# taintpro98/rnd-semantic-segmentation

Measured on AMD Instinct MI355X. Metric: train images/sec at 769x769 bf16 (DeepLabV2-ResNet101 + ASPP), higher is better.
Workload: dtype bf16; 1 GPU; train_src.py DeepLabV2-R101 bf16, 769x769 synthetic Cityscapes crops, batch 8 per GPU, 1xMI355X; global_batch=8, parallelism=dp1, weights=formula (synthetic), hip_graph_replay=False

## Files before the change

### __graft_entry__.py

```python
import os
import subprocess
import sys

ROOT = os.path.dirname(os.path.abspath(__file__))
PKG = os.path.join(ROOT, "rnd_semantic_segmentation_amd")
CSRC = os.path.join(PKG, "csrc")
LIB = os.path.join(PKG, "libmi355seg.so")
SOURCES = ["igemm_nt.hip", "igemm_pp.hip", "igemm_tn.hip", "igemm_f32.hip", "pack_aspp.hip", "upsample_ce.hip", "upsample_infer.hip", "elementwise.hip", "stem.hip", "fada.hip", "colsum.hip", "batchnorm.hip", "structure_loss.hip", "comm.hip", "gconv.hip", "gnet.hip", "gald.hip", "gf32.hip", "chain.hip", "augment.hip", "augment_pra.hip", "polyp_score.hip"]


def _headers():
    return [os.path.join(CSRC, f) for f in os.listdir(CSRC) if f.endswith(".h")] + [os.path.join(ROOT, "include", "mi355seg.h")]


def _compile_one(hipcc, src, obj):
    subprocess.run([hipcc, "--offload-arch=gfx950", "-O3", "-std=c++17", "-fPIC", "-Wno-unused-result", "-c", src, "-o", obj], check=True, cwd=CSRC)


def build(force=False):
    from concurrent.futures import ThreadPoolExecutor
    hipcc = os.environ.get("HIPCC", "/opt/rocm/bin/hipcc")
    objdir = os.path.join(ROOT, "build", "obj")
    os.makedirs(objdir, exist_ok=True)
    hdr_t = max(os.path.getmtime(h) for h in _headers())
    jobs, objs = [], []
    for s in SOURCES:
        src, obj = os.path.join(CSRC, s), os.path.join(objdir, s.replace(".hip", ".o"))
        objs.append(obj)
        if force or not os.path.exists(obj) or os.path.getmtime(obj) < max(os.path.getmtime(src), hdr_t):
            jobs.append((src, obj))
    if jobs:
        with ThreadPoolExecutor(max_workers=min(len(jobs), max(1, (os.cpu_count() or 2) - 1))) as ex:
            for f in [ex.submit(_compile_one, hipcc, a, b) for a, b in jobs]:
                f.result()
    if jobs or not os.path.exists(LIB) or os.path.getmtime(LIB) < max(os.path.getmtime(o) for o in objs):
        subprocess.run([hipcc, "--offload-arch=gfx950", "-shared", "-fPIC", "-o", LIB] + objs + ["-ldl"], check=True, cwd=CSRC)
    if ROOT not in sys.path:
        sys.path.insert(0, ROOT)
    import rnd_semantic_segmentation_amd
    from rnd_semantic_segmentation_amd import _lib
    assert _lib.lib().mi_version() >= 100
# ... 47 lines not shown
```

### include/mi355seg.h

```cpp
#ifndef MI355SEG_H
#define MI355SEG_H

#include <stddef.h>
#include <stdint.h>

#ifdef __cplusplus
extern "C" {
#endif

#define MI355SEG_VERSION 100

#define MI_OK 0
#define MI_EINVAL (-22)
#define MI_ENOMEM (-12)
#define MI_EHIP (-5)

#define MI_EPI_SCALE_BIAS 1
#define MI_EPI_RESIDUAL 2
#define MI_EPI_RELU 4
#define MI_EPI_MASK 8
#define MI_EPI_OUT_F32 16
#define MI_EPI_ZSPLIT 32
#define MI_EPI_WRITE_MASK 64
#define MI_EPI_LEAKY 256
// ... 109 lines not shown
size_t mi_upsample_tversky_bce_workspace(int B, int h, int w, int H, int W);
int mi_upsample_tversky_bce(const float* low, const float* mask, float* loss_out , float* dlow, float* sums ,
                            int B, int h, int w, int H, int W, float alpha, float eps, float w_tversky, float w_bce, float grad_scale,
                            int align_corners, void* workspace, size_t workspace_bytes, void* stream);

int mi_upsample_softmax(const float* low, float* probs, uint8_t* pred, int B, int h, int w, int K, int H, int W, void* stream);

typedef struct { const float* low; int h, w; int mirror; } MiProbSource;
int mi_upsample_softmax_multi(const MiProbSource* src, int n, float* probs, int K, int H, int W, float div_a, float div_b, void* stream);

int mi_upsample_predict_score(const MiProbSource* src, int n, int K, int H, int W, float div_a, float div_b, const int64_t* labels,
                              int ignore_index, float threshold, uint8_t* pred, uint8_t* pseudo, int64_t* counts, void* stream);

int mi_upsample_predict_score_cw(const MiProbSource* src, int n, int K, int H, int W, float div_a, float div_b, const int64_t* labels,
                                 int ignore_index, const float* class_threshold, uint8_t* pred, uint8_t* pseudo, int64_t* counts, int bins,
                                 int64_t* hist, void* stream);

#define MI_POLYP_SUMS 24
#define MI_POLYP_COUNTS 4
size_t mi_polyp_score_workspace(int B, int h, int w, int H, int W);
int mi_polyp_score(const float* low, const int64_t* labels, int B, int h, int w, int H, int W, int64_t* hist, double* sums, int64_t* counts,
                   float* prob, uint8_t* pred, void* workspace, size_t workspace_bytes, void* stream);

int mi_image_resize_ac(const float* x, float* out, int B, int C, int H, int W, int Ho, int Wo, int with_mirror, void* stream);

int mi_sgd_step(float* p, const float* g, float* buf, size_t n, float lr, float momentum, float weight_decay, void* stream);
int mi_sgd_step_dev(float* p, const float* g, float* buf, size_t n, const float* hyper , void* stream);

int mi_stem_pool_fwd(const void* y, const float* scale, const float* shift, void* pool, uint8_t* idx,
                     int B, int Hc, int Wc, int C, int Hp, int Wp, void* stream);
int mi_stem_pool_bwd(const void* dpool, const uint8_t* idx, const float* scale, void* dy,
                     int B, int Hc, int Wc, int C, int Hp, int Wp, void* stream);
int mi_stem_im2col(const void* x_bf16_nhwc, void* col_bf16, int B, int H, int W, int Ho, int Wo, int ncols, void* stream);

int mi_bias_grad_bf16(const void* dy_bf16, float* db, int M, int N, int accumulate,
                      void* workspace , size_t workspace_bytes, void* stream);
size_t mi_upsample_softce_workspace(int B, int h, int w, int K, int H, int W);
int mi_upsample_softce(const float* seg_low, float inv_temperature, float clip, const float* d_low, int ldD, int domain,
                       float* loss_out, float* dd_low, int B, int h, int w, int K, int H, int W, float grad_scale,
                       void* workspace, size_t workspace_bytes, void* stream);
size_t mi_upsample_softce_2grid_workspace(int B, int hd, int wd, int K, int H, int W);
int mi_upsample_softce_2grid(const float* seg_low, int hs, int ws, int seg_align_corners, float inv_temperature, float clip,
                             const float* d_low, int hd, int wd, int ldD, int d_align_corners, int domain, float grad_scale,
                             float* loss_out, float* dd_low, int B, int K, int H, int W, void* workspace, size_t workspace_bytes, void* stream);
int mi_adam_step(float* p, const float* g, float* exp_avg, float* exp_avg_sq, size_t n, float lr, float beta1, float beta2,
                 float eps, int step, void* stream);
int mi_adam_step_clamped(float* p, float* g, float* exp_avg, float* exp_avg_sq, size_t n, float lr, float beta1, float beta2,
                         float eps, int step, float grad_clamp, void* stream);

int mi_adam_step_dev(float* p, float* g, float* exp_avg, float* exp_avg_sq, size_t n, const float* hyper , void* stream);

int mi_pack_weight_f32(const float* w_oihw, float* wp, int O, int I, int ksize, void* stream);
int mi_conv_f32(const float* a, const float* wp, float* out, int B, int Ha, int Wa, int Ca, int Ho, int Wo, int N,
                int ksize, int stride, int pad, int dil, const float* scale, const float* bias, const float* res,
                int flags, void* stream);
int mi_stem_f32(const float* x_nchw, const float* w, const float* scale, const float* shift, float* y_nhwc,
                int B, int H, int W, void* stream);
int mi_maxpool_f32(const float* y_nhwc, float* pool_nhwc, int B, int Hc, int Wc, int C, void* stream);

int mi_comm_unique_id(void* id128 );
int mi_comm_init_rank(void** comm , int nranks, const void* id128 , int rank);
int mi_comm_destroy(void* comm);
int mi_allreduce_bucket(void* ptr, size_t count, int dtype, int average, void* comm, void* stream);

int mi_relu_mask(const void* x_bf16, const void* msk, void* y_bf16, size_t n, int bits, void* stream);
int mi_frozen_bn_fold(const float* w, const float* b, const float* mean, const float* var, float* scale, float* shift, int n, void* stream);
// ... 156 lines not shown
```

### rnd_semantic_segmentation_amd/_lib.py

```python
import ctypes
import os

import torch
from ctypes import c_char_p, c_double, c_float, c_int, c_long, c_size_t, c_void_p

_HERE = os.path.dirname(os.path.abspath(__file__))
LIB_PATH = os.environ.get("MI355SEG_LIB") or os.path.join(_HERE, "libmi355seg.so")
HEADER_PATH = os.path.join(os.path.dirname(_HERE), "include", "mi355seg.h")

P, I, F, Z, L = c_void_p, c_int, c_float, c_size_t, c_long

SIGNATURES = {
    "mi_version": (I, []),
    "mi_last_error": (c_char_p, []),
    "mi_pack_weight_fwd": (I, [P, P, I, I, I, P]),
    "mi_pack_weight_dgrad": (I, [P, P, P, I, I, I, P]),
    "mi_pack_weights_multi": (I, [P, P, P, P, P, I, I, P]),
    "mi_conv_gemm": (I, [P, P, P] + [I] * 12 + [P, P, P, P, P, I, I, F, P]),
    "mi_conv_gemm_route": (I, [I] * 10),
    "mi_conv_gemm_plan": (I, [I] * 13 + [P]),
    "mi_conv_gemm_pp": (I, [P, P, P] + [I] * 12 + [P, P, P, P, P, I, I, F, I, P]),
    "mi_conv_chain": (I, [P] * 6 + [L, I, I, I] + [P] * 8 + [I, I, P]),
    "mi_conv_wgrad_workspace": (Z, [I] * 6),
    "mi_conv_wgrad_route": (I, [I] * 12),
# ... 3 lines not shown
    "mi_conv_wgrad_partial": (I, [P, P, P] + [I] * 11 + [P, I, I, I, Z, P, Z, P, P]),
    "mi_conv_wgrad_reduce": (I, [P, I, P]),
    "mi_aspp_pack_fwd": (I, [P, P, I, I, P]),
    "mi_aspp_pack_dgrad": (I, [P, P, I, I, P]),
    "mi_aspp_col2im": (I, [P, P, P, I, I, I, I, P, P]),
    "mi_aspp_im2col": (I, [P, P, I, I, I, I, P, P]),
    "mi_colsum_workspace": (Z, [I, I]),
    "mi_aspp_bias_grad": (I, [P, P, I, I, I, P, Z, P]),
    "mi_upsample_ac_fwd": (I, [P, P] + [I] * 6 + [P]),
    "mi_upsample_ac_bwd": (I, [P, P] + [I] * 6 + [P]),
    "mi_ce_workspace": (Z, [I, I, I]),
    "mi_softmax_ce_fwd": (I, [P, P, P, I, I, I, I, I, P, Z, P]),
    "mi_softmax_ce_bwd": (I, [P, P, P, P, I, I, I, I, I, F, P]),
    "mi_upsample_ce_workspace": (Z, [I] * 6),
    "mi_upsample_ce": (I, [P, P, P, P] + [I] * 7 + [F, P, Z, P]),
    "mi_upsample_ce_ex": (I, [P, P, P, P] + [I] * 7 + [F, I, P, Z, P]),
    "mi_upsample_ce_w": (I, [P, P, P, P, P] + [I] * 7 + [F, F, I, P, Z, P]),
    "mi_upsample_ce_ohem_workspace": (Z, [I] * 6),
    "mi_upsample_ce_ohem": (I, [P, P, P, P, P] + [I] * 7 + [F, L, F, I, P, Z, P]),
    "mi_upsample_gdl_workspace": (Z, [I] * 6),
    "mi_upsample_gdl": (I, [P, P, P, P, P] + [I] * 8 + [F, F, I, P, Z, P]),
    "mi_upsample_tversky_bce_workspace": (Z, [I] * 5),
    "mi_upsample_tversky_bce": (I, [P, P, P, P, P] + [I] * 5 + [F] * 5 + [I, P, Z, P]),
    "mi_upsample_softmax": (I, [P, P, P] + [I] * 6 + [P]),
    "mi_upsample_softmax_multi": (I, [P, I, P, I, I, I, F, F, P]),
    "mi_upsample_predict_score": (I, [P, I, I, I, I, F, F, P, I, F, P, P, P, P]),
    "mi_upsample_predict_score_cw": (I, [P, I, I, I, I, F, F, P, I, P, P, P, P, I, P, P]),
    "mi_polyp_score_workspace": (Z, [I] * 5),
    "mi_polyp_score": (I, [P, P] + [I] * 5 + [P, P, P, P, P, P, Z, P]),
    "mi_image_resize_ac": (I, [P, P] + [I] * 7 + [P]),
    "mi_stem_pool_fwd": (I, [P, P, P, P, P] + [I] * 6 + [P]),
    "mi_stem_pool_bwd": (I, [P, P, P, P] + [I] * 6 + [P]),
    "mi_stem_im2col": (I, [P, P] + [I] * 6 + [P]),
    "mi_bias_grad_bf16": (I, [P, P, I, I, I, P, Z, P]),
    "mi_upsample_softce_workspace": (Z, [I] * 6),
    "mi_upsample_softce": (I, [P, F, F, P, I, I, P, P] + [I] * 6 + [F, P, Z, P]),
    "mi_upsample_softce_2grid_workspace": (Z, [I] * 6),
    "mi_upsample_softce_2grid": (I, [P, I, I, I, F, F, P, I, I, I, I, I, F, P, P, I, I, I, I, P, Z, P]),
    "mi_adam_step": (I, [P, P, P, P, Z, F, F, F, F, I, P]),
    "mi_adam_step_clamped": (I, [P, P, P, P, Z, F, F, F, F, I, F, P]),
    "mi_adam_step_dev": (I, [P, P, P, P, Z, P, P]),
    "mi_sgd_step": (I, [P, P, P, Z, F, F, F, P]),
    "mi_sgd_step_dev": (I, [P, P, P, Z, P, P]),
    "mi_pack_weight_f32": (I, [P, P, I, I, I, P]),
    "mi_conv_f32": (I, [P, P, P] + [I] * 11 + [P, P, P, I, P]),
    "mi_stem_f32": (I, [P, P, P, P, P, I, I, I, P]),
    "mi_maxpool_f32": (I, [P, P, I, I, I, I, P]),
    "mi_comm_unique_id": (I, [P]),
    "mi_comm_init_rank": (I, [P, I, P, I]),
    "mi_comm_destroy": (I, [P]),
    "mi_allreduce_bucket": (I, [P, Z, I, I, P, P]),
    "mi_relu_mask": (I, [P, P, P, Z, I, P]),
    "mi_frozen_bn_fold": (I, [P, P, P, P, P, P, I, P]),
    "mi_structure_loss_workspace": (Z, [I, I, I]),
    "mi_structure_loss": (I, [P, P, I, I, I, P, P, F, P, Z, P]),
    "mi_bn_workspace": (Z, [L, I]),
    "mi_bn_colsum": (I, [P, P, L, I, P, P, Z, P]),
    "mi_bn_apply": (I, [P, P, P, P, P, P, P, I, L, I, P]),
    "mi_bn_colsum2": (I, [P, P, L, I, P, P, P, Z, P]),
    "mi_conv_gemm_stats_workspace": (Z, [L, I]),
    "mi_conv_gemm_stats": (I, [P, P, P] + [I] * 11 + [P, P, P, Z, P, P, P, P, P, F, F, P, P]),
    "mi_bn_finalize": (I, [P, P, P, c_double, P, P, P, P, P, F, F, P, I, P]),
    "mi_bn_bwd_colsums": (I, [P, P, P, P, P, L, I, P, P, P, Z, P]),
    "mi_bn_bwd_apply": (I, [P, P, P, P, P, P, P, F, P, P, L, I, P]),
    "mi_gconv_pack_elems": (Z, [I] * 4),
    "mi_gconv_pack_multi": (I, [P, P, P, P, I, I, P]),
# ... 95 lines not shown
```

### rnd_semantic_segmentation_amd/csrc/elementwise.hip

```cpp
#include "mi_common.h"
#include <mutex>
#include <stdlib.h>
#include <string.h>

static thread_local char g_err[512] = "";

int mi_set_error(int code, const char* fmt, ...) {
    va_list ap;
    va_start(ap, fmt);
    vsnprintf(g_err, sizeof(g_err), fmt, ap);
    va_end(ap);
    return code;
}

const MiSwitches& mi_sw() {
    static MiSwitches sw;
    static std::once_flag once;
    std::call_once(once, [] {
        auto env = [](const char* name, int dflt) {
            const char* e = getenv(name);
            return e ? atoi(e) : dflt;
        };
        sw.igemm_staged = env("MI_IGEMM_STAGED", 1);
        sw.igemm_pp = env("MI_IGEMM_PP", 1);
// ... 12 lines not shown
        sw.wgrad_q3_slots_beside = env("MI_WGRAD_Q3_SLOTS_BESIDE", 448);
        sw.wgrad_s4_slots = env("MI_WGRAD_S4_SLOTS", 512);
        if (sw.wgrad_s4_slots < 64) sw.wgrad_s4_slots = 512;
        sw.wgrad_ti256 = env("MI_WGRAD_TI256", -1);
        sw.wgrad_p3 = env("MI_WGRAD_P3", 0);
        sw.wgrad_q3 = env("MI_WGRAD_Q3", 1);
        sw.wgrad_s4 = env("MI_WGRAD_S4", 1);
        sw.gconv_bn128 = env("MI_GCONV_BN128", 0);
        sw.gconv_kc = env("MI_GCONV_KC", 0);
        sw.gconv_remap = env("MI_GCONV_REMAP", 1);
        sw.gconv_ks2_wgs = env("MI_GCONV_KS2_WGS", 320);
        sw.gconv_kc32_wgs = env("MI_GCONV_KC32_WGS", 1536);
        sw.gconv_bn32_wgs = env("MI_GCONV_BN32_WGS", 256);
        sw.gconv_bn_any = env("MI_GCONV_BN_ANY", 1);
        sw.gconv_bn_c = env("MI_GCONV_BN_C", 64);
        sw.gconv_bn_force = env("MI_GCONV_BN_FORCE", 0);
        sw.gconv3_wgs = env("MI_GCONV3_WGS", 512);
#ifdef MI_EXPERIMENTS
        sw.gconv_dbg = env("MI_GC_DBG", 0);
        sw.gw_dbg = env("MI_GW_DBG", 0);
#else
        sw.gconv_dbg = sw.gw_dbg = 0;
#endif
        sw.gwm_steps = env("MI_GWM_STEPS", 48);
        if (sw.gwm_steps < 1) sw.gwm_steps = 48;
        sw.gwm_fused3 = env("MI_GWM_FUSED3", 1);
        sw.gwgrad3 = env("MI_GWGRAD3", 1);
#ifdef MI_EXPERIMENTS
        sw.p3_dbg = env("MI_P3_DBG", 0);
#else
        sw.p3_dbg = 0;
#endif
        sw.pp_trace_wg = env("MI_PP_TRACE_WG", 0);
    });
    return sw;
}

extern "C" int mi_version(void) { return MI355SEG_VERSION; }
extern "C" const char* mi_last_error(void) { return g_err; }

namespace {

__global__ void sgd_kernel(float* __restrict__ p, const float* __restrict__ g, float* __restrict__ buf, size_t n4, size_t n, float lr,
                           float mu, float wd) {
    const size_t stride = (size_t)gridDim.x * blockDim.x;
    for (size_t i = (size_t)blockIdx.x * blockDim.x + threadIdx.x; i < n4; i += stride) {
        f32x4 pv = reinterpret_cast<f32x4*>(p)[i];
        const f32x4 gv = reinterpret_cast<const f32x4*>(g)[i];
        f32x4 bv = reinterpret_cast<f32x4*>(buf)[i];
#pragma unroll
        for (int e = 0; e < 4; ++e) {
            const float gg = gv[e] + wd * pv[e];
            bv[e] = mu * bv[e] + gg;
            pv[e] = pv[e] - lr * bv[e];
        }
        reinterpret_cast<f32x4*>(buf)[i] = bv;
        reinterpret_cast<f32x4*>(p)[i] = pv;
    }
    if (blockIdx.x == 0 && threadIdx.x < (n & 3)) {
        const size_t i = (n4 << 2) + threadIdx.x;
        const float gg = g[i] + wd * p[i];
        const float b = mu * buf[i] + gg;
        buf[i] = b;
        p[i] = p[i] - lr * b;
    }
}
// ... 112 lines not shown
```

### rnd_semantic_segmentation_amd/csrc/mi_common.h

```cpp
#pragma once
#include <hip/hip_runtime.h>
#include <stdint.h>
#include <stdio.h>
#include <stdarg.h>
#include <atomic>
#include "../../include/mi355seg.h"

typedef __attribute__((ext_vector_type(8))) __bf16 bf16x8;
typedef __attribute__((ext_vector_type(4))) __bf16 bf16x4;
typedef __attribute__((ext_vector_type(2))) __bf16 bf16x2;
typedef __attribute__((ext_vector_type(4))) float f32x4;
typedef __attribute__((ext_vector_type(4))) short s16x4;
typedef __attribute__((ext_vector_type(4))) uint32_t u32x4;
typedef __attribute__((ext_vector_type(2))) uint32_t u32x2;

int mi_set_error(int code, const char* fmt, ...);

struct MiSwitches {
    int igemm_staged;
    int igemm_pp;
    int igemm_pp_mink;
    int igemm_mt;
    int igemm_bn;
    int igemm_pref;
    int pp_korder;
    int pp_loop;
    int igemm_pw;
    int wgrad_q3_slots;
    int wgrad_q3_slots_beside;
    int wgrad_s4_slots;
    int wgrad_ti256;
    int wgrad_p3;
    int wgrad_q3;
    int wgrad_s4;
    int gconv_bn128;
    int gconv_kc;
    int gconv_remap;
    int gconv_ks2_wgs;
    int gconv_kc32_wgs;
    int gconv_bn32_wgs;
    int gconv_bn_any;
    int gconv_bn_c;
    int gconv_bn_force;
    int gconv3_wgs;
    int gconv_dbg;
    int gw_dbg;
    int gwm_steps;
    int gwm_fused3;
    int gwgrad3;
    int p3_dbg;
    int pp_trace_wg;
};
const MiSwitches& mi_sw();

struct MiConvStats {
    float* partial;
    const float* pilot;
    int nparts;
};
int mi_conv_gemm_impl(const void* a, const void* wp, void* out, int B, int Ha, int Wa, int Ca, int Ho, int Wo, int N, int ksize, int stride, int pad,
                      int dil, int gather_mode, const float* scale, const float* bias, const void* res, const void* msk, void* mask_out, int flags,
                      int zgw, float alpha, void* stream, MiConvStats* st);
int mi_conv_gemm_pp_impl(const void* a, const void* wp, void* out, int B, int Ha, int Wa, int Ca, int Ho, int Wo, int N, int ksize, int stride, int pad,
                         int dil, int gather_mode, const float* scale, const float* bias, const void* res, const void* msk, void* mask_out, int flags,
                         int zgw, float alpha, int mtg, void* stream, MiConvStats* st);
struct MiConvPlan {
    int kernel;
    int mt;
    int bn;
    int unit, pref, staged;
    int epi;
    int korder;
    int m_tiles, n_tiles;
    int slots, rounds;
};
int mi_conv_plan(int B, int Ha, int Wa, int Ca, int Ho, int Wo, int N, int ksize, int stride, int pad, int dil, int flags, int pp_mtg, MiConvPlan* pl);
struct MiBnFinal {
    const float* pilot;
    double count;
    const float* gamma;
    const float* beta;
    float* running_mean;
    float* running_var;
    long long* num_batches_tracked;
// ... 93 lines not shown
```

### rnd_semantic_segmentation_amd/host/engine.py

```python
import contextlib
import os

import torch

from .. import kernels as K
from . import arch


class FlatStore:

    ALIGN = 64

    def __init__(self, named_params, device):
        self.names = [n for n, _ in named_params]
        self.params = [p for _, p in named_params]
        self.offsets = []
        off = 0
        for p in self.params:
            self.offsets.append(off)
            off += -(-p.numel() // self.ALIGN) * self.ALIGN
        self.total = off
        self.data = torch.zeros(off, dtype=torch.float32, device=device)
        self.grad = torch.zeros(off, dtype=torch.float32, device=device)
        self.written = set()
# ... 556 lines not shown
            c1, c2, c3 = arch.block_convs(blk)[:3]
            a1 = self._conv(y, c1, True)
            a2 = self._conv(a1, c2, True)
            idn = self._conv(y, arch.block_convs(blk)[3], False) if blk.down else y
            y = self._conv(a2, c3, True, res=idn)
        return y


class Fp32Aspp:

    def __init__(self, owner, rates):
        self.owner, self.rates = owner, rates
        self._sig = None

    def prepare(self):
        convs = [getattr(self.owner.conv2d_list, str(i)) for i in range(4)]
        store = getattr(convs[0].weight, "_mi_store", None)
        sig = (store.generation if store is not None else -1, sum(c.weight._version + c.bias._version for c in convs), convs[0].weight.data_ptr())
        if sig != self._sig:
            self._wp = [K.pack_weight_f32(c.weight.detach().contiguous()) for c in convs]
            self._b = [c.bias.detach().contiguous() for c in convs]
            self._sig = sig

    def forward(self, x):
        self.prepare()
        h, w = x.shape[1], x.shape[2]
        out = None
        for wp, b, d in zip(self._wp, self._b, self.rates):
            out = K.conv_f32(x, wp, (h, w), 3, 1, d, d, bias=b, res=out)
        return out


def stem_conv_forward(x, weight):
    y, col = K.stem_conv_fwd(x, weight)
    return y, (col,)


def stem_conv_wgrad(dy_nhwc, saved):
    return K.stem_wgrad(dy_nhwc, col=saved[0])


class StemConvFn(torch.autograd.Function):

    @staticmethod
    def forward(ctx, x, weight):
        y, saved = stem_conv_forward(x, weight)
        ctx.save_for_backward(*saved)
        return y

    @staticmethod
    def backward(ctx, dy):
        return None, stem_conv_wgrad(dy.contiguous(), ctx.saved_tensors)


class StemFn(torch.autograd.Function):

    @staticmethod
    def forward(ctx, x, weight, scale, shift):
        y, saved = stem_conv_forward(x, weight)
        pool, idx = K.stem_pool_fwd(y, scale, shift)
        ctx.save_for_backward(idx, scale, *saved)
        ctx.conv_hw = (y.shape[1], y.shape[2])
        return pool

    @staticmethod
    def backward(ctx, dpool):
        idx, scale = ctx.saved_tensors[:2]
        dy = K.stem_pool_bwd(dpool.contiguous(), idx, scale, ctx.conv_hw)
        return None, stem_conv_wgrad(dy, ctx.saved_tensors[2:]), None, None


# ... 197 lines not shown
```

### rnd_semantic_segmentation_amd/host/modules.py

```python
import logging
import os

import torch
import torch.nn as nn
import torch.nn.functional as F

from .. import _lib
from . import arch, engine


class FrozenBatchNorm2d(nn.Module):

    def __init__(self, n):
        super().__init__()
        self.register_buffer("weight", torch.ones(n))
        self.register_buffer("bias", torch.zeros(n))
        self.register_buffer("running_mean", torch.zeros(n))
        self.register_buffer("running_var", torch.ones(n))

    def fold(self):
        scale = self.weight * self.running_var.rsqrt()
        return scale, self.bias - self.running_mean * scale

    def forward(self, x):
# ... 65 lines not shown

    def engine_parameters(self):
        return [(k, p) for k, p in self.named_parameters()]

    def ensure_flat(self):
        dev = self.backbone.conv1.weight.device
        if self._store is None or not self._store.intact() or self._store.data.device != dev:
            self._store = engine.FlatStore(self.engine_parameters(), dev)
        return self._store

    def _stem_fold(self):
        bn = self.backbone.bn1
        sig = (engine.bn_versions(bn), bn.weight.data_ptr())
        if getattr(self, "_stem_sig", None) != sig:
            self._stem_scale, self._stem_shift = engine.bn_fold(bn)
            self._stem_sig = sig
        return self._stem_scale, self._stem_shift

    def sync_batchnorm(self, on=True):
        for m in self.backbone.modules():
            if isinstance(m, nn.BatchNorm2d):
                m._mi_sync = bool(on)
        return self

    def forward(self, x):
        _require_gpu(x, "resnet_feature_extractor")
        if self.precision == "fp32":
            if torch.is_grad_enabled() and any(p.requires_grad for p in self.parameters()):
                raise _lib.MiError("the fp32 path is forward-only (evaluation): call it under torch.no_grad(), or "
                                   "set_precision('bf16') to train")
            return self._fp32.forward(x.float()).permute(0, 3, 1, 2)
        self.ensure_flat()
        bb = self.backbone
        xb = x.to(dtype=torch.bfloat16).contiguous(memory_format=torch.channels_last)
        self._engine.batch_stats = (not self.freeze_bn) and self.training
        if self._engine.batch_stats:
            y = engine.BnStemFn.apply(xb, bb.conv1.weight, bb.bn1.weight, bb.bn1.bias, bb.bn1)
            params = [p for rt in self._engine.convs for p in (rt.weight, rt.bn.weight, rt.bn.bias)]
            return engine.BnStagesFn.apply(y, self._engine, *params).permute(0, 3, 1, 2)
        scale, shift = self._stem_fold()
        y = engine.StemFn.apply(xb, bb.conv1.weight, scale, shift)
        weights = [rt.weight for rt in self._engine.convs]
        feat = engine.StagesFn.apply(y, self._engine, *weights)
        return feat.permute(0, 3, 1, 2)


class ASPP_Classifier_V2(nn.Module):

    def __init__(self, in_channels, dilation_series, padding_series, num_classes):
        super().__init__()
        if list(dilation_series) != list(padding_series) or len(dilation_series) != 4:
            raise NotImplementedError("ASPP engine expects 4 branches with padding == dilation (build.py:26-28 passes "
                                      "[6, 12, 18, 24] twice)")
        self.in_channels, self.num_classes = in_channels, num_classes
        self.rates = tuple(int(d) for d in dilation_series)
        self.conv2d_list = arch.Holder()
        for i in range(4):
            node = arch.Holder()
            node.weight = nn.Parameter(torch.randn(num_classes, in_channels, 3, 3) * 0.01)
            self.conv2d_list.add_module(str(i), node)
        bound = 1.0 / (in_channels * 9) ** 0.5
        for i in range(4):
            getattr(self.conv2d_list, str(i)).bias = nn.Parameter(torch.empty(num_classes).uniform_(-bound, bound))
        self._engine = engine.AsppEngine(self, self.rates, num_classes, in_channels)
        self._fp32 = engine.Fp32Aspp(self, self.rates)
        self.precision = "bf16"
        self._store = None
# ... 145 lines not shown
```

### rnd_semantic_segmentation_amd/kernels.py

```python
import collections
import ctypes

import torch

from . import _lib
from ._lib import check

EPI_SCALE_BIAS, EPI_RESIDUAL, EPI_RELU, EPI_MASK, EPI_OUT_F32, EPI_ZSPLIT, EPI_WRITE_MASK, EPI_BITMASK, EPI_LEAKY = 1, 2, 4, 8, 16, 32, 64, 128, 256
GATHER_FWD, GATHER_DGRAD = 0, 1
ASPP_ZGW, ASPP_KPAD = 20, 704


def _stream():
    return ctypes.c_void_p(torch.cuda.current_stream().cuda_stream)


PROFILE = None


def _timed(name, flops, launch, tag=None):
    if PROFILE is None:
        return launch()
    e0, e1 = torch.cuda.Event(enable_timing=True), torch.cuda.Event(enable_timing=True)
    e0.record()
# ... 626 lines not shown

def stem_im2col(x, ncols):
    _chk_dtype = x.dtype
    if _chk_dtype != torch.bfloat16 or not x.is_cuda:
        raise _lib.MiError("stem_im2col: x must be a bf16 GPU tensor")
    B, _, H, W = x.shape
    Ho, Wo = (H + 6 - 7) // 2 + 1, (W + 6 - 7) // 2 + 1
    xn = x.permute(0, 2, 3, 1)
    if not xn.is_contiguous():
        xn = xn.contiguous()
    col = torch.empty((B, Ho, Wo, ncols), dtype=torch.bfloat16, device=x.device)
    check(_lib.lib().mi_stem_im2col(_p(xn), _p(col), B, H, W, Ho, Wo, ncols, _stream()), "mi_stem_im2col")
    return col


def stem_conv_fwd(x, weight):
    col = stem_im2col(x, 192)
    O = weight.shape[0]
    wp = torch.zeros((1, O, 192), dtype=torch.bfloat16, device=x.device)
    wp[0, :, :147] = weight.detach().reshape(O, 147).to(torch.bfloat16)
    return conv_gemm(col, wp, (col.shape[1], col.shape[2]), 1, 1, 0, 1, GATHER_FWD), col


def stem_wgrad(dy, x=None, col=None):
    _chk(dy, torch.bfloat16, "dy")
    if col is None:
        col = stem_im2col(x, 160)
    O, n = dy.shape[-1], col.shape[-1]
    dw = torch.empty((O, n, 1, 1), dtype=torch.float32, device=dy.device)
    conv_wgrad(dy, col, dw, 1, 1, 0, 1)
    return dw.view(O, n)[:, :147].reshape(O, 3, 7, 7)


def bias_grad_bf16(dy, db, accumulate=False):
    _chk(dy, torch.bfloat16, "dy")
    _chk(db, torch.float32, "db")
    N = dy.shape[-1]
    L = _lib.lib()
    ws = _workspace(L.mi_colsum_workspace(dy.numel() // N, N), dy.device, "colsum")
    check(L.mi_bias_grad_bf16(_p(dy), _p(db), dy.numel() // N, N, int(accumulate), _p(ws), ws.numel(), _stream()), "mi_bias_grad_bf16")
    return db


def upsample_softce(seg_low, d_low, size, domain, temperature=1.8, clip=0.9, want_grad=True, grad_scale=1.0):
    _chk(seg_low, torch.float32, "seg_low")
    _chk(d_low, torch.float32, "d_low")
    B, h, w, Kc = seg_low.shape
    ldD = d_low.shape[-1]
    H, W = size
    L = _lib.lib()
    ws = _workspace(L.mi_upsample_softce_workspace(B, h, w, Kc, H, W), seg_low.device, "softce")
    out = torch.empty(2, dtype=torch.float32, device=seg_low.device)
    dd = torch.empty_like(d_low) if want_grad else None
    check(L.mi_upsample_softce(_p(seg_low), 1.0 / float(temperature), float(clip), _p(d_low), ldD, int(domain), _p(out), _p(dd), B, h, w, Kc,
                               H, W, float(grad_scale), _p(ws), ws.numel(), _stream()), "mi_upsample_softce")
    return out, dd


def upsample_softce_2grid(seg_low, d_low, size, domain, temperature=1.8, clip=0.9, want_grad=True, grad_scale=1.0, seg_align_corners=False,
                          d_align_corners=True):
    _chk(seg_low, torch.float32, "seg_low")
    _chk(d_low, torch.float32, "d_low")
    B, hs, ws, Kc = seg_low.shape
    Bd, hd, wd, ldD = d_low.shape
    if Bd != B:
        raise _lib.MiError("upsample_softce_2grid: seg_low holds %d images, d_low %d" % (B, Bd))
# ... 254 lines not shown
```

Measured before the change: 302.3 images/s.

## Replace im2col stem conv with direct LDS-tiled MFMA forward and wgrad kernels

New measurement: 307.1 images/s (median of 6 runs). 1.02x the previous value.

```diff
diff --git a/__graft_entry__.py b/__graft_entry__.py
--- a/__graft_entry__.py
+++ b/__graft_entry__.py
@@ -6,7 +6,7 @@
 PKG = os.path.join(ROOT, "rnd_semantic_segmentation_amd")
 CSRC = os.path.join(PKG, "csrc")
 LIB = os.path.join(PKG, "libmi355seg.so")
-SOURCES = ["igemm_nt.hip", "igemm_pp.hip", "igemm_tn.hip", "igemm_f32.hip", "pack_aspp.hip", "upsample_ce.hip", "upsample_infer.hip", "elementwise.hip", "stem.hip", "fada.hip", "colsum.hip", "batchnorm.hip", "structure_loss.hip", "comm.hip", "gconv.hip", "gnet.hip", "gald.hip", "gf32.hip", "chain.hip", "augment.hip", "augment_pra.hip", "polyp_score.hip"]
+SOURCES = ["igemm_nt.hip", "igemm_pp.hip", "igemm_tn.hip", "igemm_f32.hip", "pack_aspp.hip", "upsample_ce.hip", "upsample_infer.hip", "elementwise.hip", "stem.hip", "stem_direct.hip", "fada.hip", "colsum.hip", "batchnorm.hip", "structure_loss.hip", "comm.hip", "gconv.hip", "gnet.hip", "gald.hip", "gf32.hip", "chain.hip", "augment.hip", "augment_pra.hip", "polyp_score.hip"]
 
 
 def _headers():
diff --git a/include/mi355seg.h b/include/mi355seg.h
--- a/include/mi355seg.h
+++ b/include/mi355seg.h
@@ -165,6 +165,12 @@
 int mi_stem_pool_bwd(const void* dpool, const uint8_t* idx, const float* scale, void* dy,
                      int B, int Hc, int Wc, int C, int Hp, int Wp, void* stream);
 int mi_stem_im2col(const void* x_bf16_nhwc, void* col_bf16, int B, int H, int W, int Ho, int Wo, int ncols, void* stream);
+int mi_stem_direct_enabled(void);
+int mi_stem_pack_image(const void* x, int x_is_bf16_nhwc, void* x4, int B, int H, int W, void* stream);
+int mi_stem_conv_fwd(const void* x4, const float* w, void* wpack, void* y, int B, int H, int W, int O, int Ho, int Wo, void* stream);
+size_t mi_stem_conv_wgrad_workspace(int B, int Ho, int Wo);
+int mi_stem_conv_wgrad(const void* dy, const void* x4, float* dw, int B, int H, int W, int O, int Ho, int Wo, void* workspace,
+                       size_t workspace_bytes, void* stream);
 
 int mi_bias_grad_bf16(const void* dy_bf16, float* db, int M, int N, int accumulate,
                       void* workspace , size_t workspace_bytes, void* stream);
diff --git a/rnd_semantic_segmentation_amd/_lib.py b/rnd_semantic_segmentation_amd/_lib.py
--- a/rnd_semantic_segmentation_amd/_lib.py
+++ b/rnd_semantic_segmentation_amd/_lib.py
@@ -59,6 +59,11 @@
     "mi_stem_pool_fwd": (I, [P, P, P, P, P] + [I] * 6 + [P]),
     "mi_stem_pool_bwd": (I, [P, P, P, P] + [I] * 6 + [P]),
     "mi_stem_im2col": (I, [P, P] + [I] * 6 + [P]),
+    "mi_stem_direct_enabled": (I, []),
+    "mi_stem_pack_image": (I, [P, I, P, I, I, I, P]),
+    "mi_stem_conv_fwd": (I, [P, P, P, P] + [I] * 6 + [P]),
+    "mi_stem_conv_wgrad_workspace": (Z, [I] * 3),
+    "mi_stem_conv_wgrad": (I, [P, P, P] + [I] * 6 + [P, Z, P]),
     "mi_bias_grad_bf16": (I, [P, P, I, I, I, P, Z, P]),
     "mi_upsample_softce_workspace": (Z, [I] * 6),
     "mi_upsample_softce": (I, [P, F, F, P, I, I, P, P] + [I] * 6 + [F, P, Z, P]),
diff --git a/rnd_semantic_segmentation_amd/csrc/elementwise.hip b/rnd_semantic_segmentation_amd/csrc/elementwise.hip
--- a/rnd_semantic_segmentation_amd/csrc/elementwise.hip
+++ b/rnd_semantic_segmentation_amd/csrc/elementwise.hip
@@ -68,6 +68,9 @@
         sw.p3_dbg = 0;
 #endif
         sw.pp_trace_wg = env("MI_PP_TRACE_WG", 0);
+        sw.stem_direct = env("MI_STEM_DIRECT", 1);
+        sw.stem_wgrad_splits = env("MI_STEM_WGRAD_SPLITS", 512);
+        if (sw.stem_wgrad_splits < 1 || sw.stem_wgrad_splits > 4096) sw.stem_wgrad_splits = 512;
     });
     return sw;
 }
diff --git a/rnd_semantic_segmentation_amd/csrc/mi_common.h b/rnd_semantic_segmentation_amd/csrc/mi_common.h
--- a/rnd_semantic_segmentation_amd/csrc/mi_common.h
+++ b/rnd_semantic_segmentation_amd/csrc/mi_common.h
@@ -50,6 +50,8 @@
     int gwgrad3;
     int p3_dbg;
     int pp_trace_wg;
+    int stem_wgrad_splits;
+    int stem_direct;
 };
 const MiSwitches& mi_sw();
 
diff --git a/rnd_semantic_segmentation_amd/csrc/stem_direct.hip b/rnd_semantic_segmentation_amd/csrc/stem_direct.hip
--- /dev/null
+++ b/rnd_semantic_segmentation_amd/csrc/stem_direct.hip
@@ -0,0 +1,382 @@
+#include "mi_common.h"
+
+namespace {
+
+constexpr int SD_TW = 64;
+constexpr int SD_ROWPX = 136;
+constexpr int SD_ROWB = SD_ROWPX * 8;
+constexpr int SD_FWD_TH = 8;
+constexpr int SD_FWD_ROWS = 2 * SD_FWD_TH + 5;
+constexpr int SD_KB = 6;
+constexpr int SD_WG_TH = 4;
+constexpr int SD_WG_ROWS = 2 * SD_WG_TH + 5;
+constexpr int SD_DYROWB = SD_TW * 128;
+constexpr int SD_PART = 64 * 7 * 32;
+
+__global__ __launch_bounds__(256) void stem_pack_f32_kernel(const float* __restrict__ x, bf16x4* __restrict__ x4, long HW, int B) {
+    const int b = blockIdx.y;
+    const float* img = x + (long)b * 3 * HW;
+    const long p0 = (long)blockIdx.x * 1024 + threadIdx.x;
+    float v[4][3];
+#pragma unroll
+    for (int j = 0; j < 4; ++j) {
+        const long p = p0 + j * 256;
+#pragma unroll
+        for (int c = 0; c < 3; ++c) v[j][c] = p < HW ? img[c * HW + p] : 0.f;
+    }
+#pragma unroll
+    for (int j = 0; j < 4; ++j) {
+        const long p = p0 + j * 256;
+        if (p < HW) {
+            bf16x4 o;
+            o[0] = (__bf16)v[j][0];
+            o[1] = (__bf16)v[j][1];
+            o[2] = (__bf16)v[j][2];
+            o[3] = (__bf16)0.f;
+            x4[(long)b * HW + p] = o;
+        }
+    }
+}
+
+__global__ __launch_bounds__(256) void stem_pack_bf16_kernel(const __bf16* __restrict__ x, bf16x4* __restrict__ x4, long n) {
+    const long p = (long)blockIdx.x * 256 + threadIdx.x;
+    if (p >= n) return;
+    bf16x4 o;
+    o[0] = x[p * 3];
+    o[1] = x[p * 3 + 1];
+    o[2] = x[p * 3 + 2];
+    o[3] = (__bf16)0.f;
+    x4[p] = o;
+}
+
+__global__ __launch_bounds__(256) void stem_pack_weight_kernel(const float* __restrict__ w, __bf16* __restrict__ wp) {
+    const int i = blockIdx.x * 256 + threadIdx.x;
+    if (i >= SD_KB * 64 * 32) return;
+    const int kk = i & 31, o = (i >> 5) & 63, kb = i >> 11;
+    const int k = kb * 32 + kk;
+    wp[i] = (__bf16)(k < 147 ? w[o * 147 + k] : 0.f);
+}
+
+template <int ROWS>
+struct ImageRows {
+    static constexpr int N = (ROWS * SD_ROWPX + 255) / 256;
+    uint2 v[N];
+    __device__ __forceinline__ void load(const uint2* __restrict__ img, int h0, int c0, int H, int W, int tid) {
+#pragma unroll
+        for (int j = 0; j < N; ++j) {
+            const int i = tid + j * 256;
+            const int r = i / SD_ROWPX, c = i - r * SD_ROWPX;
+            const int h = h0 + r, w = c0 + c;
+            v[j] = make_uint2(0u, 0u);
+            if (i < ROWS * SD_ROWPX && (unsigned)h < (unsigned)H && (unsigned)w < (unsigned)W) v[j] = img[(long)h * W + w];
+        }
+    }
+    __device__ __forceinline__ void store(uint2* sx, int tid) const {
+#pragma unroll
+        for (int j = 0; j < N; ++j) {
+            const int i = tid + j * 256;
+            if (i < ROWS * SD_ROWPX) sx[i] = v[j];
+        }
+    }
+};
+
+struct StemFwdParams {
+    const uint2* x4;
+    const bf16x8* wp;
+    __bf16* y;
+    int B, H, W, Ho, Wo, tiles_x, tiles_y;
+};
+
+__global__ __launch_bounds__(256, 2) void stem_direct_fwd_kernel(StemFwdParams p) {
+    __shared__ __attribute__((aligned(16))) uint2 sx[SD_FWD_ROWS * SD_ROWPX];
+    const int tid = threadIdx.x, lane = tid & 63;
+    const int wave = __builtin_amdgcn_readfirstlane(tid >> 6);
+    const int tx = blockIdx.x % p.tiles_x, ty = (blockIdx.x / p.tiles_x) % p.tiles_y, b = blockIdx.x / (p.tiles_x * p.tiles_y);
+    const int wo0 = tx * SD_TW, ho0 = ty * SD_FWD_TH;
+    ImageRows<SD_FWD_ROWS> rows;
+    rows.load(p.x4 + (long)b * p.H * p.W, 2 * ho0 - 3, 2 * wo0 - 3, p.H, p.W, tid);
+
+    const int col = lane & 15, q = lane >> 4;
+    bf16x8 wf[SD_KB - 1][4];
+#pragma unroll
+    for (int kb = 0; kb < SD_KB - 1; ++kb)
+#pragma unroll
+        for (int ot = 0; ot < 4; ++ot) wf[kb][ot] = p.wp[(kb * 64 + (col >> 2) * 16 + ot * 4 + (col & 3)) * 4 + q];
+    int off[SD_KB - 1][8];
+#pragma unroll
+    for (int kb = 0; kb < SD_KB - 1; ++kb)
+#pragma unroll
+        for (int j = 0; j < 8; ++j) {
+            const int k = kb * 32 + q * 8 + j;
+            const int c = k / 49, r = k - c * 49, ky = r / 7, kx = r - ky * 7;
+            off[kb][j] = k < 147 ? ky * SD_ROWB + kx * 8 + c * 2 : -1;
+        }
+    rows.store(sx, tid);
+    __syncthreads();
+
+    const char* sxb = reinterpret_cast<const char*>(sx);
+    bf16x8 zero8;
+#pragma unroll
+    for (int e = 0; e < 8; ++e) zero8[e] = (__bf16)0.f;
+    for (int rr = wave * 2; rr < wave * 2 + 2; ++rr) {
+        const int ho = ho0 + rr;
+        if (ho >= p.Ho) break;
+        for (int mt = 0; mt < 4; ++mt) {
+            if (wo0 + mt * 16 >= p.Wo) break;
+            const char* win = sxb + 2 * rr * SD_ROWB + 16 * (mt * 16 + col);
+            f32x4 acc[4];
+#pragma unroll
+            for (int ot = 0; ot < 4; ++ot) acc[ot] = f32x4{0.f, 0.f, 0.f, 0.f};
+#pragma unroll
+            for (int kb = 0; kb < SD_KB - 1; ++kb) {
+                union { bf16x8 v; unsigned short s[8]; } f;
+#pragma unroll
+                for (int j = 0; j < 8; ++j) {
+                    if (kb < 4) {
+                        f.s[j] = *reinterpret_cast<const unsigned short*>(win + off[kb][j]);
+                    } else {
+                        const unsigned short v = *reinterpret_cast<const unsigned short*>(win + (off[kb][j] < 0 ? 0 : off[kb][j]));
+                        f.s[j] = off[kb][j] < 0 ? (unsigned short)0 : v;
+                    }
+                }
+#pragma unroll
+                for (int ot = 0; ot < 4; ++ot) acc[ot] = __builtin_amdgcn_mfma_f32_16x16x32_bf16(wf[kb][ot], f.v, acc[ot], 0, 0, 0);
+            }
+#pragma unroll
+            for (int ot = 0; ot < 4; ++ot) acc[ot] = __builtin_amdgcn_mfma_f32_16x16x32_bf16(zero8, zero8, acc[ot], 0, 0, 0);
+            const int wo = wo0 + mt * 16 + col;
+            if (wo < p.Wo) {
+                bf16x8 o0, o1;
+#pragma unroll
+                for (int e = 0; e < 4; ++e) {
+                    o0[e] = (__bf16)acc[0][e];
+                    o0[4 + e] = (__bf16)acc[1][e];
+                    o1[e] = (__bf16)acc[2][e];
+                    o1[4 + e] = (__bf16)acc[3][e];
+                }
+                bf16x8* dst = reinterpret_cast<bf16x8*>(p.y + (((long)b * p.Ho + ho) * p.Wo + wo) * 64 + q * 16);
+                dst[0] = o0;
+                dst[1] = o1;
+            }
+        }
+    }
+}
+
+template <int OFF>
+__device__ __forceinline__ s16x4 sd_tr_read(unsigned lds_addr) {
+    s16x4 v;
+    asm volatile("ds_read_b64_tr_b16 %0, %1 offset:%2" : "=v"(v) : "v"(lds_addr), "n"(OFF));
+    return v;
+}
+
+__device__ __forceinline__ unsigned sd_lds_address(const void* generic_ptr_into_lds) {
+    return (unsigned)(uintptr_t)((__attribute__((address_space(3))) const char*)generic_ptr_into_lds);
+}
+
+struct StemWgradParams {
+    const uint2* x4;
+    const bf16x8* dy;
+    float* part;
+    int B, H, W, Ho, Wo, tiles_x, tiles_y, tiles, S;
+};
+
+__global__ __launch_bounds__(256, 2) void stem_direct_wgrad_kernel(StemWgradParams p) {
+    __shared__ __attribute__((aligned(16))) uint2 sx[SD_WG_ROWS * SD_ROWPX];
+    __shared__ __attribute__((aligned(16))) bf16x8 sdy[SD_WG_TH * SD_TW * 8];
+    const int tid = threadIdx.x, lane = tid & 63;
+    const int wave = __builtin_amdgcn_readfirstlane(tid >> 6);
+    const int kt = wave & 1, oh = wave >> 1;
+    const int s = blockIdx.x;
+    const int t_begin = (int)((long)s * p.tiles / p.S), t_end = (int)((long)(s + 1) * p.tiles / p.S);
+    const int g = lane >> 4, rq = (lane & 15) >> 2, pc = lane & 3;
+    const int pix = 4 * g + rq;
+    const unsigned sx_base = sd_lds_address(sx) + 16 * pix + 32 * kt + 8 * pc;
+    const unsigned sdy_base = sd_lds_address(sdy) + 128 * pix + 8 * (pc & 1);
+    const int sw = pix & 7;
+
+    f32x4 acc[2][7];
+#pragma unroll
+    for (int a = 0; a < 2; ++a)
+#pragma unroll
+        for (int ky = 0; ky < 7; ++ky) acc[a][ky] = f32x4{0.f, 0.f, 0.f, 0.f};
+
+    ImageRows<SD_WG_ROWS> nx;
+    bf16x8 ny[8];
+    auto load_tile = [&](int t) {
+        const int tx = t % p.tiles_x, ty = (t / p.tiles_x) % p.tiles_y, b = t / (p.tiles_x * p.tiles_y);
+        const int wo0 = tx * SD_TW, ho0 = ty * SD_WG_TH;
+        nx.load(p.x4 + (long)b * p.H * p.W, 2 * ho0 - 3, 2 * wo0 - 3, p.H, p.W, tid);
+#pragma unroll
+        for (int j = 0; j < 8; ++j) {
+            const int i = tid + j * 256;
+            const int c = i & 7, P = (i >> 3) & 63, rr = i >> 9;
+            const int ho = ho0 + rr, wo = wo0 + P;
+#pragma unroll
+            for (int e = 0; e < 8; ++e) ny[j][e] = (__bf16)0.f;
+            if (ho < p.Ho && wo < p.Wo) ny[j] = p.dy[(((long)b * p.Ho + ho) * p.Wo + wo) * 8 + c];
+        }
+    };
+    load_tile(t_begin);
+    for (int t = t_begin; t < t_end; ++t) {
+        const int tx = t % p.tiles_x, ty = (t / p.tiles_x) % p.tiles_y;
+        const int wo0 = tx * SD_TW, ho0 = ty * SD_WG_TH;
+        __syncthreads();
+        nx.store(sx, tid);
+#pragma unroll
+        for (int j = 0; j < 8; ++j) {
+            const int i = tid + j * 256;
+            const int c = i & 7, P = (i >> 3) & 63, rr = i >> 9;
+            sdy[(rr * SD_TW + P) * 8 + (c ^ (P & 7))] = ny[j];
+        }
+        __syncthreads();
+        if (t + 1 < t_end) load_tile(t + 1);
+        const int nrows = min(SD_WG_TH, p.Ho - ho0);
+        for (int rr = 0; rr < nrows; ++rr) {
+#pragma unroll
+            for (int step = 0; step < 2; ++step) {
+                const int left = p.Wo - (wo0 + step * 32);
+                if (left <= 0) break;
+                union { bf16x8 v; s16x4 h[2]; uint64_t d[2]; } yf[2], xf[7];
+                const unsigned ya = sdy_base + rr * SD_DYROWB + step * 32 * 128;
+#pragma unroll
+                for (int a = 0; a < 2; ++a) {
+                    const unsigned addr = ya + (((2 * (oh * 2 + a) + (pc >> 1)) ^ sw) << 4);
+                    yf[a].h[0] = sd_tr_read<0>(addr);
+                    yf[a].h[1] = sd_tr_read<16 * 128>(addr);
+                }
+                const unsigned xa = sx_base + 2 * rr * SD_ROWB + step * 32 * 16;
+#pragma unroll
+                for (int ky = 0; ky < 7; ++ky) {
+                    xf[ky].h[0] = sd_tr_read<0>(xa + ky * SD_ROWB);
+                    xf[ky].h[1] = sd_tr_read<16 * 16>(xa + ky * SD_ROWB);
+                }
+                asm volatile("s_waitcnt lgkmcnt(0)" ::: "memory");
+                __builtin_amdgcn_sched_barrier(0);
+                if (left < 32) {
+#pragma unroll
+                    for (int h = 0; h < 2; ++h) {
+                        const int nv = left - (16 * h + 4 * g);
+                        const uint64_t m = nv >= 4 ? ~0ull : (nv <= 0 ? 0ull : ((1ull << (16 * nv)) - 1ull));
+#pragma unroll
+                        for (int ky = 0; ky < 7; ++ky) xf[ky].d[h] &= m;
+                    }
+                }
+#pragma unroll
+                for (int ky = 0; ky < 7; ++ky)
+#pragma unroll
+                    for (int a = 0; a < 2; ++a) acc[a][ky] = __builtin_amdgcn_mfma_f32_16x16x32_bf16(yf[a].v, xf[ky].v, acc[a][ky], 0, 0, 0);
+            }
+        }
+    }
+    float* dst = p.part + (long)s * SD_PART;
+#pragma unroll
+    for (int a = 0; a < 2; ++a)
+#pragma unroll
+        for (int ky = 0; ky < 7; ++ky)
+#pragma unroll
+            for (int e = 0; e < 4; ++e) dst[(((oh * 2 + a) * 16 + 4 * g + e) * 7 + ky) * 32 + kt * 16 + (lane & 15)] = acc[a][ky][e];
+}
+
+__global__ __launch_bounds__(256) void stem_direct_wgrad_reduce_kernel(const float* __restrict__ part, float* __restrict__ dw, int S) {
+    const int i = blockIdx.x * 256 + threadIdx.x;
+    if (i >= SD_PART) return;
+    const int k = i & 31, ky = (i >> 5) % 7, o = i / 224;
+    const int kx = k >> 2, c = k & 3;
+    if (c == 3 || kx >= 7) return;
+    float sum = 0.f;
+    int s = 0;
+    for (; s + 64 <= S; s += 64) {
+        float v[64];
+#pragma unroll
+        for (int j = 0; j < 64; ++j) v[j] = part[(long)(s + j) * SD_PART + i];
+#pragma unroll
+        for (int j = 0; j < 64; ++j) sum += v[j];
+    }
+    for (; s < S; ++s) sum += part[(long)s * SD_PART + i];
+    dw[((o * 3 + c) * 7 + ky) * 7 + kx] = sum;
+}
+
+int stem_wgrad_splits(int B, int Ho, int Wo) {
+    const long tiles = (long)B * ((Ho + SD_WG_TH - 1) / SD_WG_TH) * ((Wo + SD_TW - 1) / SD_TW);
+    const long slots = mi_sw().stem_wgrad_splits;
+    return (int)(tiles < slots ? tiles : slots);
+}
+
+const char* stem_direct_geometry(int B, int H, int W, int Ho, int Wo) {
+    if (B <= 0 || H <= 0 || W <= 0) return "B, H, W must be positive";
+    if (Ho != (H + 6 - 7) / 2 + 1 || Wo != (W + 6 - 7) / 2 + 1) return "output size must be that of a 7x7/2/3 conv";
+    if ((long)B * H * W * 4 >= (1l << 31) || (long)B * Ho * Wo * 64 >= (1l << 31)) return "tensor exceeds the 32-bit offset range";
+    return nullptr;
+}
+
+}
+
+extern "C" int mi_stem_direct_enabled(void) { return mi_sw().stem_direct != 0; }
+
+extern "C" int mi_stem_pack_image(const void* x, int x_is_bf16_nhwc, void* x4, int B, int H, int W, void* stream) {
+    MI_REQUIRE(x && x4 && B > 0 && H > 0 && W > 0, "mi_stem_pack_image: bad argument");
+    MI_REQUIRE(x_is_bf16_nhwc == 0 || x_is_bf16_nhwc == 1, "mi_stem_pack_image: x_is_bf16_nhwc=%d (0: fp32 NCHW, 1: bf16 NHWC)", x_is_bf16_nhwc);
+    MI_REQUIRE((reinterpret_cast<uintptr_t>(x4) & 7) == 0 && (reinterpret_cast<uintptr_t>(x) & (x_is_bf16_nhwc ? 1 : 3)) == 0, "mi_stem_pack_image: alignment");
+    MI_REQUIRE((long)B * H * W * 4 < (1l << 31), "mi_stem_pack_image: tensor exceeds the 32-bit offset range");
+    MI_REQUIRE(B < 65536, "mi_stem_pack_image: B = %d exceeds the grid", B);
+    const long HW = (long)H * W;
+    if (x_is_bf16_nhwc)
+        hipLaunchKernelGGL(stem_pack_bf16_kernel, dim3((unsigned)((B * HW + 255) / 256)), dim3(256), 0, (hipStream_t)stream, (const __bf16*)x, (bf16x4*)x4,
+                           B * HW);
+    else
+        hipLaunchKernelGGL(stem_pack_f32_kernel, dim3((unsigned)((HW + 1023) / 1024), (unsigned)B), dim3(256), 0, (hipStream_t)stream, (const float*)x,
+                           (bf16x4*)x4, HW, B);
+    MI_CHECK_LAUNCH("mi_stem_pack_image");
+    return MI_OK;
+}
+
+extern "C" int mi_stem_conv_fwd(const void* x4, const float* w, void* wpack, void* y, int B, int H, int W, int O, int Ho, int Wo, void* stream) {
+    MI_REQUIRE(x4 && w && wpack && y, "mi_stem_conv_fwd: null operand");
+    MI_REQUIRE(O == 64, "mi_stem_conv_fwd: O=%d (the stem has 64 output channels)", O);
+    const char* bad = stem_direct_geometry(B, H, W, Ho, Wo);
+    MI_REQUIRE(!bad, "mi_stem_conv_fwd: %s", bad);
+    MI_REQUIRE((reinterpret_cast<uintptr_t>(x4) & 7) == 0 && mi_aligned16(wpack) && mi_aligned16(y), "mi_stem_conv_fwd: alignment");
+    hipLaunchKernelGGL(stem_pack_weight_kernel, dim3(SD_KB * 64 * 32 / 256), dim3(256), 0, (hipStream_t)stream, w, (__bf16*)wpack);
+    MI_CHECK_LAUNCH("mi_stem_conv_fwd (weight pack)");
+    StemFwdParams p;
+    p.x4 = (const uint2*)x4;
+    p.wp = (const bf16x8*)wpack;
+    p.y = (__bf16*)y;
+    p.B = B, p.H = H, p.W = W, p.Ho = Ho, p.Wo = Wo;
+    p.tiles_x = (Wo + SD_TW - 1) / SD_TW;
+    p.tiles_y = (Ho + SD_FWD_TH - 1) / SD_FWD_TH;
+    hipLaunchKernelGGL(stem_direct_fwd_kernel, dim3((unsigned)(B * p.tiles_x * p.tiles_y)), dim3(256), 0, (hipStream_t)stream, p);
+    MI_CHECK_LAUNCH("mi_stem_conv_fwd");
+    return MI_OK;
+}
+
+extern "C" size_t mi_stem_conv_wgrad_workspace(int B, int Ho, int Wo) {
+    if (B <= 0 || Ho <= 0 || Wo <= 0) return 0;
+    return (size_t)stem_wgrad_splits(B, Ho, Wo) * SD_PART * sizeof(float);
+}
+
+extern "C" int mi_stem_conv_wgrad(const void* dy, const void* x4, float* dw, int B, int H, int W, int O, int Ho, int Wo, void* workspace,
+                                  size_t workspace_bytes, void* stream) {
+    MI_REQUIRE(dy && x4 && dw && workspace, "mi_stem_conv_wgrad: null operand");
+    MI_REQUIRE(O == 64, "mi_stem_conv_wgrad: O=%d (the stem has 64 output channels)", O);
+    const char* bad = stem_direct_geometry(B, H, W, Ho, Wo);
+    MI_REQUIRE(!bad, "mi_stem_conv_wgrad: %s", bad);
+    MI_REQUIRE((reinterpret_cast<uintptr_t>(x4) & 7) == 0 && mi_aligned16(dy) && mi_aligned16(workspace) && (reinterpret_cast<uintptr_t>(dw) & 3) == 0,
+               "mi_stem_conv_wgrad: alignment");
+    MI_REQUIRE(workspace_bytes >= mi_stem_conv_wgrad_workspace(B, Ho, Wo), "mi_stem_conv_wgrad: workspace holds %zu bytes, %zu needed", workspace_bytes,
+               mi_stem_conv_wgrad_workspace(B, Ho, Wo));
+    StemWgradParams p;
+    p.x4 = (const uint2*)x4;
+    p.dy = (const bf16x8*)dy;
+    p.part = (float*)workspace;
+    p.B = B, p.H = H, p.W = W, p.Ho = Ho, p.Wo = Wo;
+    p.tiles_x = (Wo + SD_TW - 1) / SD_TW;
+    p.tiles_y = (Ho + SD_WG_TH - 1) / SD_WG_TH;
+    p.tiles = B * p.tiles_x * p.tiles_y;
+    p.S = stem_wgrad_splits(B, Ho, Wo);
+    hipLaunchKernelGGL(stem_direct_wgrad_kernel, dim3((unsigned)p.S), dim3(256), 0, (hipStream_t)stream, p);
+    MI_CHECK_LAUNCH("mi_stem_conv_wgrad");
+    hipLaunchKernelGGL(stem_direct_wgrad_reduce_kernel, dim3(SD_PART / 256), dim3(256), 0, (hipStream_t)stream, (const float*)workspace, dw, p.S);
+    MI_CHECK_LAUNCH("mi_stem_conv_wgrad (reduce)");
+    return MI_OK;
+}
diff --git a/rnd_semantic_segmentation_amd/host/engine.py b/rnd_semantic_segmentation_amd/host/engine.py
--- a/rnd_semantic_segmentation_amd/host/engine.py
+++ b/rnd_semantic_segmentation_amd/host/engine.py
@@ -612,11 +612,16 @@
 
 
 def stem_conv_forward(x, weight):
-    y, col = K.stem_conv_fwd(x, weight)
+    if K.stem_direct_enabled():
+        x4 = K.stem_pack_image(x)
+        return K.stem_conv_direct(x4, weight), (x4,)
+    y, col = K.stem_conv_fwd(x.to(dtype=torch.bfloat16).contiguous(memory_format=torch.channels_last), weight)
     return y, (col,)
 
 
 def stem_conv_wgrad(dy_nhwc, saved):
+    if K.stem_direct_enabled():
+        return K.stem_wgrad_direct(dy_nhwc, saved[0])
     return K.stem_wgrad(dy_nhwc, col=saved[0])
 
 
diff --git a/rnd_semantic_segmentation_amd/host/modules.py b/rnd_semantic_segmentation_amd/host/modules.py
--- a/rnd_semantic_segmentation_amd/host/modules.py
+++ b/rnd_semantic_segmentation_amd/host/modules.py
@@ -121,7 +121,7 @@
             return self._fp32.forward(x.float()).permute(0, 3, 1, 2)
         self.ensure_flat()
         bb = self.backbone
-        xb = x.to(dtype=torch.bfloat16).contiguous(memory_format=torch.channels_last)
+        xb = x
         self._engine.batch_stats = (not self.freeze_bn) and self.training
         if self._engine.batch_stats:
             y = engine.BnStemFn.apply(xb, bb.conv1.weight, bb.bn1.weight, bb.bn1.bias, bb.bn1)
diff --git a/rnd_semantic_segmentation_amd/kernels.py b/rnd_semantic_segmentation_amd/kernels.py
--- a/rnd_semantic_segmentation_amd/kernels.py
+++ b/rnd_semantic_segmentation_amd/kernels.py
@@ -682,6 +682,63 @@
     return dw.view(O, n)[:, :147].reshape(O, 3, 7, 7)
 
 
+def stem_direct_enabled():
+    return bool(_lib.lib().mi_stem_direct_enabled())
+
+
+def _stem_out_hw(H, W):
+    return (H + 6 - 7) // 2 + 1, (W + 6 - 7) // 2 + 1
+
+
+def stem_pack_image(x):
+    if not x.is_cuda:
+        raise _lib.MiError("stem_pack_image: x must live on the GPU (no CPU path exists)")
+    if x.dim() != 4 or x.shape[1] != 3:
+        raise _lib.MiError("stem_pack_image: x must be [B,3,H,W], got %s" % (tuple(x.shape),))
+    B, _, H, W = x.shape
+    if x.dtype == torch.float32 and x.is_contiguous():
+        src, nhwc = x, 0
+    else:
+        src = x.to(dtype=torch.bfloat16).permute(0, 2, 3, 1)
+        if not src.is_contiguous():
+            src = src.contiguous()
+        nhwc = 1
+    x4 = torch.empty((B, H, W, 4), dtype=torch.bfloat16, device=x.device)
+    check(_lib.lib().mi_stem_pack_image(_p(src), nhwc, _p(x4), B, H, W, _stream()), "mi_stem_pack_image")
+    return x4
+
+
+def stem_conv_direct(x4, weight):
+    _chk(x4, torch.bfloat16, "x4")
+    w = _chk(weight.detach(), torch.float32, "weight")
+    B, H, W, C4 = x4.shape
+    if C4 != 4 or tuple(w.shape[1:]) != (3, 7, 7):
+        raise _lib.MiError("stem_conv_direct: x4 %s, weight %s" % (tuple(x4.shape), tuple(w.shape)))
+    O = w.shape[0]
+    Ho, Wo = _stem_out_hw(H, W)
+    y = torch.empty((B, Ho, Wo, O), dtype=torch.bfloat16, device=x4.device)
+    wpack = _workspace(6 * 64 * 32 * 2, x4.device, "stem_wpack")
+    check(_timed("stem_direct_fwd_kernel", 2.0 * B * Ho * Wo * O * 147, lambda: _lib.lib().mi_stem_conv_fwd(
+        _p(x4), _p(w), _p(wpack), _p(y), B, H, W, O, Ho, Wo, _stream()), tag=("fwd", 7, 4, O, B * Ho * Wo, 0, 1)), "mi_stem_conv_fwd")
+    return y
+
+
+def stem_wgrad_direct(dy, x4):
+    _chk(dy, torch.bfloat16, "dy")
+    _chk(x4, torch.bfloat16, "x4")
+    B, H, W, C4 = x4.shape
+    Ho, Wo = _stem_out_hw(H, W)
+    O = dy.shape[-1]
+    if C4 != 4 or tuple(dy.shape[:3]) != (B, Ho, Wo):
+        raise _lib.MiError("stem_wgrad_direct: dy %s does not belong to x4 %s" % (tuple(dy.shape), tuple(x4.shape)))
+    L = _lib.lib()
+    dw = torch.empty((O, 3, 7, 7), dtype=torch.float32, device=dy.device)
+    ws = _workspace(L.mi_stem_conv_wgrad_workspace(B, Ho, Wo), dy.device, "stem_wgrad")
+    check(_timed("stem_direct_wgrad_kernel+reduce", 2.0 * B * Ho * Wo * O * 147, lambda: L.mi_stem_conv_wgrad(
+        _p(dy), _p(x4), _p(dw), B, H, W, O, Ho, Wo, _p(ws), ws.numel(), _stream()), tag=("wgrad", 7, 4, O, B * Ho * Wo, 0, 1)), "mi_stem_conv_wgrad")
+    return dw
+
+
 def bias_grad_bf16(dy, db, accumulate=False):
     _chk(dy, torch.bfloat16, "dy")
     _chk(db, torch.float32, "db")
```
